# xvjiarui/VFS

Hardware: AMD Instinct MI355X
Metric: frame-pairs/sec (train) R50 256² (higher is better)
Workload: dtype bf16; 1 GPU; ResNet-50 SimSiam (VFS) forward_train+backward+SGD, imgs [32,2,3,1,256,256] per GPU (configs[2] shape), SyncBN, fp32 master weights; parallelism=dp1

## Files before the change

vfs_amd/csrc/stem.hip:

```cpp
#include "vfs_conv.h"
#include "vfs_ops.h"
#include "vfs_stem.h"

#define OOB_OFFSET 0xFFFFFFF0u
typedef __attribute__((ext_vector_type(4))) short s16x4;

#define ST_PH 21
#define ST_PW 38
#define ST_PROW (ST_PW * 4)

__device__ __forceinline__ int stem_w_off(int r, int cout, int chunk) {
  return (r * 64 + cout) * 32 + ((chunk ^ ((cout >> 2) & 3)) << 3);
}

#define ST_STAGE_ROW 72
__global__ __launch_bounds__(256) void stem_fwd_direct_kernel(ConvArgs a, int tiles_per_block, int ntiles) {
  __shared__ __attribute__((aligned(16))) bf16_t sW[7 * 64 * 32];
  __shared__ __attribute__((aligned(16))) bf16_t sX[ST_PH * ST_PROW];
  __shared__ __attribute__((aligned(16))) bf16_t sOut[4 * 32 * ST_STAGE_ROW];
  auto sred = [&](int w) { return reinterpret_cast<float*>(sOut + w * (32 * ST_STAGE_ROW)); };
  constexpr int PL = (ST_PH * 19 + 255) / 256;
  const ConvGeom g = a.g;
  const int t = threadIdx.x, lane = t & 63, wp = t >> 6;
  const int lr = lane & 15, lq = lane >> 4;
  const int tiles_x = (g.Wo + 15) / 16, tiles_y = (g.Ho + 7) / 8, tiles_img = tiles_x * tiles_y;

  for (int i = t; i < 7 * 64 * 4; i += 256) {
    const int chunk = i & 3, cout = (i >> 2) & 63, r = i >> 8;
    st16(&sW[stem_w_off(r, cout, chunk)], ld16(a.wgt + ((size_t)cout * 8 + r) * 32 + chunk * 8));
  }
  const __amdgpu_buffer_rsrc_t xrs = __builtin_amdgcn_make_buffer_rsrc(
      (void*)a.src, 0, (unsigned)((size_t)g.N * g.H * g.W * 4 * 2), 0x00020000);

  u32x4 pr_[PL];
  auto load_patch = [&](int tile) {
    const int tx = tile % tiles_x, ty = (tile / tiles_x) % tiles_y, n = tile / tiles_img;
#pragma unroll
    for (int k = 0; k < PL; ++k) {
      const int i = t + 256 * k;
      const int prow = i / 19, pc = i - prow * 19;
      const int y = 2 * ty * 8 - 3 + prow, x = 2 * tx * 16 - 4 + 2 * pc;
      const bool ok = i < ST_PH * 19 && (unsigned)y < (unsigned)g.H && (unsigned)x < (unsigned)g.W;
      const unsigned off = ok ? (unsigned)((((size_t)(n * g.H + y) * g.W + x) * 4) * 2) : OOB_OFFSET;
      pr_[k] = __builtin_amdgcn_raw_buffer_load_b128(xrs, off, 0, 0);
    }
  };
  auto store_patch = [&]() {
#pragma unroll
    for (int k = 0; k < PL; ++k) {
      const int i = t + 256 * k;
      if (i < ST_PH * 19) {
        const int prow = i / 19, pc = i - prow * 19;
        st16(&sX[prow * ST_PROW + pc * 8], pr_[k]);
      }
    }
  };

  const int t_begin = blockIdx.x * tiles_per_block, t_end = min(ntiles, t_begin + tiles_per_block);
  if (t_begin >= t_end) return;
  const bool do_stats = a.stats != nullptr;
  float s1[4][4], s2[4][4];
#pragma unroll
  for (int tm = 0; tm < 4; ++tm)
#pragma unroll
    for (int q = 0; q < 4; ++q) { s1[tm][q] = 0.f; s2[tm][q] = 0.f; }
  int run_first = t_begin;
  load_patch(t_begin);
  store_patch();
  __syncthreads();
  bf16_t* slab = sOut + wp * (32 * ST_STAGE_ROW);
  for (int tile = t_begin; tile < t_end; ++tile) {
    const int tx = tile % tiles_x, ty = (tile / tiles_x) % tiles_y, n = tile / tiles_img;
    const int y0 = ty * 8, x0 = tx * 16;
    const bool has_next = tile + 1 < t_end;
    if (has_next) load_patch(tile + 1);
    __builtin_amdgcn_sched_barrier(0);
    f32x4 acc[4][2];
#pragma unroll
    for (int tm = 0; tm < 4; ++tm)
#pragma unroll
      for (int tn = 0; tn < 2; ++tn) acc[tm][tn] = (f32x4){0.f, 0.f, 0.f, 0.f};
#pragma unroll
    for (int r = 0; r < 7; ++r) {
      bf16x8 af[4], bfr[2];
#pragma unroll
      for (int tm = 0; tm < 4; ++tm)
        af[tm] = *reinterpret_cast<const bf16x8*>(&sW[stem_w_off(r, tm * 16 + lr, lq)]);
#pragma unroll
      for (int tn = 0; tn < 2; ++tn) {
        const int py = wp * 2 + tn;
        bfr[tn] = *reinterpret_cast<const bf16x8*>(&sX[(2 * py + r) * ST_PROW + (2 * lr + 2 * lq) * 4]);
      }
#pragma unroll
      for (int tm = 0; tm < 4; ++tm)
#pragma unroll
        for (int tn = 0; tn < 2; ++tn)
          acc[tm][tn] = __builtin_amdgcn_mfma_f32_16x16x32_bf16(af[tm], bfr[tn], acc[tm][tn], 0, 0, 0);
    }
#pragma unroll
    for (int tn = 0; tn < 2; ++tn) {
      const bool mok = y0 + wp * 2 + tn < g.Ho && x0 + lr < g.Wo;
#pragma unroll
      for (int tm = 0; tm < 4; ++tm) {
        u32x2 pk;
        pk.x = pack2bf(acc[tm][tn][0], acc[tm][tn][1]);
        pk.y = pack2bf(acc[tm][tn][2], acc[tm][tn][3]);
        st8(&slab[(tn * 16 + lr) * ST_STAGE_ROW + tm * 16 + lq * 4], pk);
        if (do_stats && mok) {
          const float q0 = bflo(pk.x), q1 = bfhi(pk.x), q2 = bflo(pk.y), q3 = bfhi(pk.y);
          s1[tm][0] += q0; s2[tm][0] += q0 * q0;
          s1[tm][1] += q1; s2[tm][1] += q1 * q1;
          s1[tm][2] += q2; s2[tm][2] += q2 * q2;
          s1[tm][3] += q3; s2[tm][3] += q3 * q3;
        }
      }
    }
    __builtin_amdgcn_wave_barrier();
#pragma unroll
    for (int i = 0; i < 4; ++i) {
      const int p = i * 8 + (lane >> 3), ch = lane & 7;
      const int y = y0 + wp * 2 + (p >> 4), x = x0 + (p & 15);
      if (y < g.Ho && x < g.Wo)
        st16(a.out + (((size_t)n * g.Ho + y) * g.Wo + x) * 64 + ch * 8, ld16(&slab[p * ST_STAGE_ROW + ch * 8]));
    }
    const bool run_ends = !has_next || (tile + 1) / tiles_img != n;
    if (do_stats) {
      if (run_ends) {
#pragma unroll
        for (int tm = 0; tm < 4; ++tm) {
          f32x4 r1, r2;
#pragma unroll
          for (int q = 0; q < 4; ++q) {
            r1[q] = row16_sum(s1[tm][q]);
            r2[q] = row16_sum(s2[tm][q]);
            s1[tm][q] = 0.f; s2[tm][q] = 0.f;
          }
          if (lr == 0) {
            *reinterpret_cast<f32x4*>(sred(wp) + tm * 16 + lq * 4) = r1;
            *reinterpret_cast<f32x4*>(sred(wp) + 64 + tm * 16 + lq * 4) = r2;
          }
        }
        __syncthreads();
        if (t < 128) {
          const int st = t >> 6, cl = t & 63;
          const int o = st * 64 + cl;
          a.stats[(size_t)run_first * 128 + t] = (sred(0)[o] + sred(1)[o]) + (sred(2)[o] + sred(3)[o]);
        }
        if (tile != run_first && t >= 128) a.stats[(size_t)tile * 128 + (t - 128)] = 0.f;
        run_first = tile + 1;
      } else if (tile != run_first && t < 128) {
        a.stats[(size_t)tile * 128 + t] = 0.f;
      }
    }
    __syncthreads();
    if (has_next) store_patch();
    __syncthreads();
  }
}

int vfs_stem_tiles(int N, int Ho, int Wo) { return N * ((Ho + 7) / 8) * ((Wo + 15) / 16); }

int vfs_stem_fwd_direct_launch(const ConvArgs& a, hipStream_t stream) {
  const int ntiles = vfs_stem_tiles(a.g.N, a.g.Ho, a.g.Wo);
  const int maxb = vfs_option_stem_blocks > 0 ? vfs_option_stem_blocks : 2048;
  int blocks = ntiles < maxb ? ntiles : maxb;
  const int tpb = (ntiles + blocks - 1) / blocks;
  blocks = (ntiles + tpb - 1) / tpb;
  hipLaunchKernelGGL(stem_fwd_direct_kernel, dim3(blocks), dim3(256), 0, stream, a, tpb, ntiles);
  return vfs_check_launch("stem_fwd_direct");
}

#define SD_RS 72

__global__ __launch_bounds__(256) void stem_wgrad_fused_kernel(StemBwdArgs a, const bf16_t* __restrict__ x4, int Hin, int Win,
                                                               float* __restrict__ partial, int tiles_per_block,
                                                               int ntiles) {
  __shared__ __attribute__((aligned(16))) bf16_t sX[ST_PH * ST_PROW];
  __shared__ __attribute__((aligned(16))) bf16_t sD[128 * SD_RS];
  __shared__ float sTab[STEM_MAX_GROUPS * STEM_TAB];
  const int t = threadIdx.x, lane = t & 63, wave = t >> 6;
  const int wk = wave >> 1, wn = wave & 1;
  const int lr = lane & 15, lq = lane >> 4;
  const int tiles_x = (a.W + 15) / 16, tiles_y = (a.H + 7) / 8;
  const float rc = (float)(1.0 / a.count);
  stem_fill_table(a, sTab, rc);
  const __amdgpu_buffer_rsrc_t xrs = __builtin_amdgcn_make_buffer_rsrc(
      (void*)x4, 0, (unsigned)((size_t)a.N * Hin * Win * 4 * 2), 0x00020000);

  f32x4 acc[7][2];
#pragma unroll
  for (int i = 0; i < 7; ++i)
#pragma unroll
    for (int tn = 0; tn < 2; ++tn) acc[i][tn] = (f32x4){0.f, 0.f, 0.f, 0.f};

  const int pl = 4 * lq + (lr >> 2), q4 = lr & 3;
  const int d_base = pl * SD_RS + wn * 32 + q4 * 4;
  const int x_base = (2 * pl + q4) * 4;

  const int t_begin = blockIdx.x * tiles_per_block, t_end = min(ntiles, t_begin + tiles_per_block);
  for (int tile = t_begin; tile < t_end; ++tile) {
    const int tx = tile % tiles_x, ty = (tile / tiles_x) % tiles_y, n = tile / (tiles_x * tiles_y);
    const int y0 = ty * 8, x0 = tx * 16;
    __syncthreads();
    for (int i = t; i < ST_PH * 19; i += 256) {
      const int pr = i / 19, pc = i - pr * 19;
      const int y = 2 * y0 - 3 + pr, x = 2 * x0 - 4 + 2 * pc;
      const bool ok = (unsigned)y < (unsigned)Hin && (unsigned)x < (unsigned)Win;
      const unsigned off = ok ? (unsigned)((((size_t)(n * Hin + y) * Win + x) * 4) * 2) : OOB_OFFSET;
      st16(&sX[pr * ST_PROW + pc * 8], __builtin_amdgcn_raw_buffer_load_b128(xrs, off, 0, 0));
    }
#pragma unroll
    for (int i = 0; i < 4; ++i) {
      const int v = t + 256 * i, ps = v >> 3, j = v & 7;
      const int q = ps & 15, p = (ps & ~15) | (q < 8 ? 2 * q : 2 * (q - 8) + 1);
      const int y = y0 + (p >> 4), x = x0 + (p & 15);
      float d[8];
      if (y < a.H && x < a.W) {
        stem_dx_vec(a, sTab, n, y, x, j * 8, d);
      } else {
#pragma unroll
        for (int e = 0; e < 8; ++e) d[e] = 0.f;
      }
      st16(&sD[p * SD_RS + j * 8], pack8(d));
    }
    __syncthreads();
#pragma unroll
    for (int ks = 0; ks < 4; ++ks) {
      bf16x8 bfr[2];
#pragma unroll
      for (int tn = 0; tn < 2; ++tn) {
        const bf16_t* b0 = sD + d_base + (32 * ks) * SD_RS + tn * 16;
        const s16x4 lo = __builtin_amdgcn_ds_read_tr16_b64_v4i16((__attribute__((address_space(3))) s16x4*)(b0));
        const s16x4 hi = __builtin_amdgcn_ds_read_tr16_b64_v4i16((__attribute__((address_space(3))) s16x4*)(b0 + 16 * SD_RS));
        bfr[tn][0] = lo[0]; bfr[tn][1] = lo[1]; bfr[tn][2] = lo[2]; bfr[tn][3] = lo[3];
        bfr[tn][4] = hi[0]; bfr[tn][5] = hi[1]; bfr[tn][6] = hi[2]; bfr[tn][7] = hi[3];
      }
#pragma unroll
      for (int i = 0; i < 7; ++i) {
        const int rt = wk * 7 + i, r = rt >> 1, s0 = (rt & 1) * 4;
        const bf16_t* a0 = sX + x_base + (4 * ks + r) * ST_PROW + s0 * 4;
        const s16x4 lo = __builtin_amdgcn_ds_read_tr16_b64_v4i16((__attribute__((address_space(3))) s16x4*)(a0));
        const s16x4 hi = __builtin_amdgcn_ds_read_tr16_b64_v4i16((__attribute__((address_space(3))) s16x4*)(a0 + 2 * ST_PROW));
        bf16x8 af;
        af[0] = lo[0]; af[1] = lo[1]; af[2] = lo[2]; af[3] = lo[3];
        af[4] = hi[0]; af[5] = hi[1]; af[6] = hi[2]; af[7] = hi[3];
#pragma unroll
        for (int tn = 0; tn < 2; ++tn)
          acc[i][tn] = __builtin_amdgcn_mfma_f32_16x16x32_bf16(af, bfr[tn], acc[i][tn], 0, 0, 0);
      }
    }
  }
#pragma unroll
  for (int i = 0; i < 7; ++i) {
    const int rt = wk * 7 + i, r = rt >> 1, s0 = (rt & 1) * 4;
#pragma unroll
    for (int tn = 0; tn < 2; ++tn) {
      const int cout = wn * 32 + tn * 16 + lr;
      *reinterpret_cast<f32x4*>(partial + (((size_t)blockIdx.x * 64 + cout) * 7 + r) * 32 + (s0 + lq) * 4) = acc[i][tn];
    }
  }
}

int vfs_stem_wgrad_fused_launch(const StemBwdArgs& a, const bf16_t* x4, int Hin, int Win, float* partial, int nblocks,
                                hipStream_t stream) {
  const int ntiles = vfs_stem_tiles(a.N, a.H, a.W);
  if ((a.N + a.npg - 1) / a.npg > 8) return vfs_set_error(VFS_ERR_SHAPE, "stem_wgrad_fused: more than 8 BN groups");
  if ((long long)a.N * a.H * a.W * 64 >= (1ll << 31)) return vfs_set_error(VFS_ERR_SHAPE, "stem_wgrad_fused: 2^31 elements or more (32-bit offsets)");
  if (nblocks > ntiles) nblocks = ntiles;
  const int tpb = (ntiles + nblocks - 1) / nblocks;
  if ((ntiles + tpb - 1) / tpb != nblocks) return vfs_set_error(VFS_ERR_SHAPE, "stem_wgrad_fused: nblocks must equal ceil(ntiles / ceil(ntiles/nblocks))");
  hipLaunchKernelGGL(stem_wgrad_fused_kernel, dim3(nblocks), dim3(256), 0, stream, a, x4, Hin, Win, partial, tpb, ntiles);
  return vfs_check_launch("stem_wgrad_fused");
}
```

vfs_amd/csrc/vfs_options.h:

```cpp
#pragma once

#define VFS_OPTIONS(X)                                                                                                              \
                                                               \
  X(halo, 1)                                                                 \
  X(halo_min_fill, 70)         \
  X(halo_deep_max, 256)        \
  X(halo_xcd, 1)                                                           \
                                                                                                          \
  X(stem_direct, 1)                   \
  X(stem_blocks, 0)                     \
                                                                                                       \
  X(bn_ticket, 1)                      \
  X(bn_chunk_rows, 64)                 \
  X(bn_wide, 1)                \
  X(bn_wide_min_mb, 8)                                                                       \
                                                                  \
  X(igemm_bc, 0)                                                                      \
  X(igemm_xcd, 1)                                                                              \
  X(igemm_mfma_stats, 1)            \
  X(igemm_narrow_below, 513)   \
  X(igemm_onek, 3)             \
  X(igemm_ring_tiles, 512)                         \
  X(igemm_ring_fbn, 1)                        \
  X(igemm_ring_mfma32, 1)       \
  X(igemm_ring_gather, 0)      \
  X(igemm_ring_upfront, 0)                   \
  X(igemm_skinny, 1)                                  \
  X(igemm_pw, 0)               \
  X(igemm_pw_min_tiles, 192)   \
                                                                    \
  X(wgrad_lin, 1)                                               \
  X(wgrad_lin2, 1)                               \
  X(wgrad_ring, 1)             \
  X(wgrad_xcd, 1)                                              \
                                                                                     \
  X(conv_f32_variant, 0)          \
  X(conv_f32_dbg, 0)                                  \
  X(lpx_target, 0)             \
  X(lpx_wgs, 0)                \
  X(lpx_minb, 4)                                                       \
                                                                              \
  X(lp2, 1)                                                                              \
  X(lp2_dbg, 0)                \
  X(lp2_fpb, 0)                                       \
  X(lp2_trim, 1)               \
  X(lp2_cap, 0)                \
  X(lp2_xcd, -1)


#define VFS_OPTION_DECLARE(name, dflt) extern int vfs_option_##name;
VFS_OPTIONS(VFS_OPTION_DECLARE)
#undef VFS_OPTION_DECLARE
```

Baseline: 3995 frame-pairs/s.

## Add pooled-gradient stem wgrad kernel that scatters maxpool grads in shared memory

Adds a new stem weight-gradient kernel that reads the pooled-output gradient and argmax indices directly and scatters them into a per-wave shared-memory buffer via a lookup table. It then combines them with BN backward terms before the MFMA wgrad accumulation, instead of reading a pre-expanded full-resolution gradient. This is meant to cut global-memory traffic for the maxpool-backward result and possibly a separate unpool pass. In exchange it uses more shared memory and LDS read-modify-write scatter, and it relies on overlapping pool windows being handled correctly. It is enabled by default through a new option.

```diff
diff --git a/vfs_amd/csrc/stem.hip b/vfs_amd/csrc/stem.hip
--- a/vfs_amd/csrc/stem.hip
+++ b/vfs_amd/csrc/stem.hip
@@ -261,6 +261,157 @@
   }
 }
 
+#define SP_COLS 18
+#define SP_DUMP (2 * SP_COLS * 64)
+#define SP_REGION (SP_DUMP + 64)
+
+__global__ __launch_bounds__(256, 3) void stem_wgrad_fused_kernel_pooled(StemBwdArgs a, const bf16_t* __restrict__ x4, int Hin, int Win,
+                                                                float* __restrict__ partial, int tiles_per_block, int ntiles) {
+  __shared__ __attribute__((aligned(16))) bf16_t sX[ST_PH * ST_PROW];
+  __shared__ __attribute__((aligned(16))) float sC[4 * SP_REGION];
+  __shared__ float sTab[STEM_MAX_GROUPS * STEM_TAB];
+  __shared__ unsigned short sLut[2 * 256];
+  const int t = threadIdx.x, lane = t & 63, wave = t >> 6;
+  const int wk = wave >> 1, wn = wave & 1;
+  const int lr = lane & 15, lq = lane >> 4;
+  const int tiles_x = (a.W + 15) / 16, tiles_y = (a.H + 7) / 8;
+  const float rc = (float)(1.0 / a.count);
+  stem_fill_table(a, sTab, rc);
+  for (int i = t; i < 2 * 256; i += 256) {
+    const int ph = i >> 8, c = i & 255, dr = c / 3, dc = c - 3 * dr;
+    const bool ok = ph == 0 ? (c >= 3 && c < 9) : c < 3;
+    sLut[i] = (unsigned short)(ok ? ((ph == 0 ? dr - 1 : 1) * SP_COLS + dc) * 64 : 0x7fff);
+  }
+  float* R = sC + wave * SP_REGION;
+  bf16_t* D = reinterpret_cast<bf16_t*>(R);
+  R[SP_DUMP + lane] = 0.f;
+  const __amdgpu_buffer_rsrc_t xrs = __builtin_amdgcn_make_buffer_rsrc(
+      (void*)x4, 0, (unsigned)((size_t)a.N * Hin * Win * 4 * 2), 0x00020000);
+
+  f32x4 acc[7][2];
+#pragma unroll
+  for (int i = 0; i < 7; ++i)
+#pragma unroll
+    for (int tn = 0; tn < 2; ++tn) acc[i][tn] = (f32x4){0.f, 0.f, 0.f, 0.f};
+
+  const int pl = 4 * lq + (lr >> 2), q4 = lr & 3;
+  const int d_base = pl * SD_RS + wn * 32 + q4 * 4;
+  const int x_base = (2 * pl + q4) * 4;
+
+  const int t_begin = blockIdx.x * tiles_per_block, t_end = min(ntiles, t_begin + tiles_per_block);
+  for (int tile = t_begin; tile < t_end; ++tile) {
+    const int tx = tile % tiles_x, ty = (tile / tiles_x) % tiles_y, n = tile / (tiles_x * tiles_y);
+    const int y0 = ty * 8, x0 = tx * 16;
+    __syncthreads();
+    u32x4 pv[2];
+#pragma unroll
+    for (int k = 0; k < 2; ++k) {
+      const int i = t + 256 * k, pr = i / 19, pc = i - pr * 19;
+      const int y = 2 * y0 - 3 + pr, x = 2 * x0 - 4 + 2 * pc;
+      const bool ok = i < ST_PH * 19 && (unsigned)y < (unsigned)Hin && (unsigned)x < (unsigned)Win;
+      const unsigned off = ok ? (unsigned)((((size_t)(n * Hin + y) * Win + x) * 4) * 2) : OOB_OFFSET;
+      pv[k] = __builtin_amdgcn_raw_buffer_load_b128(xrs, off, 0, 0);
+    }
+    bf16_t gv[2][9];
+    unsigned cv[2][9];
+#pragma unroll
+    for (int ph = 0; ph < 2; ++ph) {
+      const int aa = (y0 >> 1) + wave + ph;
+      const unsigned orow = ((unsigned)n * (unsigned)a.Hp + (unsigned)min(aa, a.Hp - 1)) * (unsigned)a.Wp;
+#pragma unroll
+      for (int k = 0; k < 9; ++k) {
+        const int bb = (x0 >> 1) + k;
+        const unsigned o = (orow + (unsigned)min(bb, a.Wp - 1)) * 64u + (unsigned)lane;
+        gv[ph][k] = a.gp[o];
+        cv[ph][k] = a.idx[o];
+      }
+    }
+    u32x4 xv[4];
+#pragma unroll
+    for (int i = 0; i < 4; ++i) {
+      const int v = lane + 64 * i, p = v >> 3, j = v & 7;
+      const int y = min(y0 + 2 * wave + (p >> 4), a.H - 1), x = min(x0 + (p & 15), a.W - 1);
+      xv[i] = ld16(a.x + ((((unsigned)n * (unsigned)a.H + (unsigned)y) * (unsigned)a.W + (unsigned)x) * 64u + (unsigned)(j * 8)));
+    }
+#pragma unroll
+    for (int ph = 0; ph < 2; ++ph)
+#pragma unroll
+      for (int k = 0; k < 9; ++k)
+        if ((y0 >> 1) + wave + ph >= a.Hp || (x0 >> 1) + k >= a.Wp) cv[ph][k] = 0xffu;
+#pragma unroll
+    for (int i = 0; i < SP_DUMP / 256; ++i) st16(R + (lane + 64 * i) * 4, zero16());
+#pragma unroll
+    for (int k = 0; k < 2; ++k) {
+      const int i = t + 256 * k, pr = i / 19, pc = i - pr * 19;
+      if (i < ST_PH * 19) st16(&sX[pr * ST_PROW + pc * 8], pv[k]);
+    }
+    __builtin_amdgcn_wave_barrier();
+#pragma unroll
+    for (int ph = 0; ph < 2; ++ph)
+#pragma unroll
+      for (int k = 0; k < 9; ++k) {
+        const unsigned cell = min((unsigned)sLut[ph * 256 + cv[ph][k]] + (unsigned)(2 * k * 64), (unsigned)SP_DUMP) + (unsigned)lane;
+        R[cell] += bf2f(gv[ph][k]);
+      }
+    __builtin_amdgcn_wave_barrier();
+    const float* tab = sTab + (n / a.npg) * STEM_TAB;
+#pragma unroll
+    for (int i = 0; i < 4; ++i) {
+      const int v = lane + 64 * i, p = v >> 3, j = v & 7;
+      const int y = y0 + 2 * wave + (p >> 4), x = x0 + (p & 15);
+      const float* cp = R + ((p >> 4) * SP_COLS + (p & 15) + 1) * 64 + j * 8;
+      float g[8], d[8];
+      *reinterpret_cast<f32x4*>(g) = *reinterpret_cast<const f32x4*>(cp);
+      *reinterpret_cast<f32x4*>(g + 4) = *reinterpret_cast<const f32x4*>(cp + 4);
+      if (y < a.H && x < a.W) {
+        stem_dx_combine(tab + j * 8, g, xv[i], d);
+      } else {
+#pragma unroll
+        for (int e = 0; e < 8; ++e) d[e] = 0.f;
+      }
+      __builtin_amdgcn_wave_barrier();
+      st16(&D[p * SD_RS + j * 8], pack8(d));
+    }
+    __syncthreads();
+#pragma unroll
+    for (int ks = 0; ks < 4; ++ks) {
+      bf16x8 bfr[2];
+#pragma unroll
+      for (int tn = 0; tn < 2; ++tn) {
+        const bf16_t* b0 = reinterpret_cast<const bf16_t*>(sC + ks * SP_REGION) + d_base + tn * 16;
+        const s16x4 lo = __builtin_amdgcn_ds_read_tr16_b64_v4i16((__attribute__((address_space(3))) s16x4*)(b0));
+        const s16x4 hi = __builtin_amdgcn_ds_read_tr16_b64_v4i16((__attribute__((address_space(3))) s16x4*)(b0 + 16 * SD_RS));
+        bfr[tn][0] = lo[0]; bfr[tn][1] = lo[1]; bfr[tn][2] = lo[2]; bfr[tn][3] = lo[3];
+        bfr[tn][4] = hi[0]; bfr[tn][5] = hi[1]; bfr[tn][6] = hi[2]; bfr[tn][7] = hi[3];
+      }
+#pragma unroll
+      for (int i = 0; i < 7; ++i) {
+        const int rt = wk * 7 + i, r = rt >> 1, s0 = (rt & 1) * 4;
+        const bf16_t* a0 = sX + x_base + (4 * ks + r) * ST_PROW + s0 * 4;
+        const s16x4 lo = __builtin_amdgcn_ds_read_tr16_b64_v4i16((__attribute__((address_space(3))) s16x4*)(a0));
+        const s16x4 hi = __builtin_amdgcn_ds_read_tr16_b64_v4i16((__attribute__((address_space(3))) s16x4*)(a0 + 2 * ST_PROW));
+        bf16x8 af;
+        af[0] = lo[0]; af[1] = lo[1]; af[2] = lo[2]; af[3] = lo[3];
+        af[4] = hi[0]; af[5] = hi[1]; af[6] = hi[2]; af[7] = hi[3];
+#pragma unroll
+        for (int tn = 0; tn < 2; ++tn)
+          acc[i][tn] = __builtin_amdgcn_mfma_f32_16x16x32_bf16(af, bfr[tn], acc[i][tn], 0, 0, 0);
+      }
+    }
+  }
+#pragma unroll
+  for (int i = 0; i < 7; ++i) {
+    const int rt = wk * 7 + i, r = rt >> 1, s0 = (rt & 1) * 4;
+#pragma unroll
+    for (int tn = 0; tn < 2; ++tn) {
+      const int cout = wn * 32 + tn * 16 + lr;
+      *reinterpret_cast<f32x4*>(partial + (((size_t)blockIdx.x * 64 + cout) * 7 + r) * 32 + (s0 + lq) * 4) = acc[i][tn];
+    }
+  }
+}
+
+static bool stem_wgrad_takes_pooled(const StemBwdArgs& a) { return vfs_option_stem_wgrad_pooled && a.H >= 4 && a.W >= 8; }
+
 int vfs_stem_wgrad_fused_launch(const StemBwdArgs& a, const bf16_t* x4, int Hin, int Win, float* partial, int nblocks,
                                 hipStream_t stream) {
   const int ntiles = vfs_stem_tiles(a.N, a.H, a.W);
@@ -269,6 +420,10 @@
   if (nblocks > ntiles) nblocks = ntiles;
   const int tpb = (ntiles + nblocks - 1) / nblocks;
   if ((ntiles + tpb - 1) / tpb != nblocks) return vfs_set_error(VFS_ERR_SHAPE, "stem_wgrad_fused: nblocks must equal ceil(ntiles / ceil(ntiles/nblocks))");
+  if (stem_wgrad_takes_pooled(a)) {
+    hipLaunchKernelGGL(stem_wgrad_fused_kernel_pooled, dim3(nblocks), dim3(256), 0, stream, a, x4, Hin, Win, partial, tpb, ntiles);
+    return vfs_check_launch("stem_wgrad_pooled");
+  }
   hipLaunchKernelGGL(stem_wgrad_fused_kernel, dim3(nblocks), dim3(256), 0, stream, a, x4, Hin, Win, partial, tpb, ntiles);
   return vfs_check_launch("stem_wgrad_fused");
 }
diff --git a/vfs_amd/csrc/vfs_options.h b/vfs_amd/csrc/vfs_options.h
--- a/vfs_amd/csrc/vfs_options.h
+++ b/vfs_amd/csrc/vfs_options.h
@@ -9,6 +9,7 @@
                                                                                                           \
   X(stem_direct, 1)                   \
   X(stem_blocks, 0)                     \
+  X(stem_wgrad_pooled, 1)      \
                                                                                                        \
   X(bn_ticket, 1)                      \
   X(bn_chunk_rows, 64)                 \
```

Result: no change. 4004 frame-pairs/s, median of 6 (+0.2%).
